# LuoweiZhou/VLP

Hardware: AMD Instinct MI355X
Metric: samples/sec/node (COCO 100-region, seq64, bs64xN) fp16 (higher is better)
Workload: dtype f16; 1 GPU; COCO Captions fine-tune shape: BERT-base 12L, 100 regions x 2048-d, seq_len 64 (L=167), bs 64/GPU, fwd+bwd+FP16 FusedAdam, dropout 0.1, dynamic loss scale; global_batch=64, parallelism=dp1, batch_pool=8, skipped_steps=0, rccl_ranks=1, optimizer=replicated, first_leg_packed=False

## Files before the change

### include/vlp_hip.h

```cpp
#ifndef VLP_HIP_H
#define VLP_HIP_H

#include <stdint.h>

#ifdef __cplusplus
extern "C" {
#endif

#define VLP_ABI_VERSION 5

typedef enum {
    VLP_OK = 0,
    VLP_ERR_BAD_ARG = -1,
    VLP_ERR_HIP = -2,
    VLP_ERR_WORKSPACE = -3
} vlp_status;

enum { VLP_ACT_NONE = 0, VLP_ACT_GELU = 1, VLP_ACT_RELU = 2, VLP_ACT_TANH = 3,
       VLP_ACT_GELU_SAVE_GRAD = 4  };
enum { VLP_MUL_NONE = 0, VLP_MUL_GELU_GRAD = 1, VLP_MUL_RELU_MASK = 2, VLP_MUL_PLAIN = 3  };

int vlp_version(void);
const char* vlp_last_error_string(void);
int vlp_lab_build(void);
// ... 384 lines not shown

int vlp_bce_loss_fwd(const void* logits, int64_t ld, const void* labels_f32, int64_t ldl, int32_t B, int32_t N,
                     float* loss, void* stream);
int vlp_bce_loss_bwd(const void* logits, int64_t ld, const void* labels_f32, int64_t ldl, int32_t B, int32_t N,
                     const float* grad_scale, void* dlogits, int64_t ldd, void* stream);
int vlp_bce_sparse_loss_fwd(const void* logits, int64_t ld, const int32_t* ans_idx, const float* ans_score, int32_t S, int32_t B, int32_t N,
                            float* loss, void* stream);
int vlp_bce_sparse_loss_bwd(const void* logits, int64_t ld, const int32_t* ans_idx, const float* ans_score, int32_t S, int32_t B, int32_t N,
                            const float* grad_scale, void* dlogits, int64_t ldd, void* stream);
int vlp_vqa_answer_rows(const void* logits, int64_t ld, int32_t rows, int32_t N, int32_t first_col, const int32_t* ans_idx,
                        const float* ans_score, int32_t S, int64_t* out_ids, float* out_vals, float* out_scores, void* stream);

int vlp_sumsq(const void* g_f16, int64_t n, float* out2, float* partial, void* stream);
int vlp_sumsq_acc(const void* g_f16, int64_t n, float* out2, float* partial, void* stream);

typedef struct {
    float* p32; float* m; float* v;
    const void* g16;
    void* p16;
    int64_t n;
    float b1, b2, eps, decay;
    int32_t eps_inside_sqrt;
    const float* hyper;
} vlp_fused_adam_args;
int vlp_fused_adam(const vlp_fused_adam_args* a, void* stream);
int vlp_adam_hyper(const float* sumsq2, const float* any_overflow, const float* scale_state, float max_grad_norm,
                   float step_size, float* hyper3, void* stream);
int vlp_loss_scale_update(float* scale_state, const float* overflow, void* stream);

int64_t vlp_bert_adam_norms_floats(int64_t n, int32_t ntensors);
typedef struct {
    float* p32; float* m; float* v;
    const void* g; int32_t g_is_f32;
    void* p16;
    const int64_t* seg_off; int32_t ntensors; int64_t n;
    float* norms; int64_t norms_floats;
    float lr, b1, b2, eps, decay, max_grad_norm;
    float grad_scale;
// ... 9 lines not shown
```

### vlp_amd/_lib.py

```python
import ctypes as C
import os

import torch

_HERE = os.path.dirname(os.path.abspath(__file__))
LIB_PATH = os.environ.get("VLP_HIP_LIB") or os.path.join(_HERE, "libvlp_hip.so")

ACT_NONE, ACT_GELU, ACT_RELU, ACT_TANH, ACT_GELU_SAVE_GRAD = 0, 1, 2, 3, 4
MUL_NONE, MUL_GELU_GRAD, MUL_RELU_MASK, MUL_PLAIN = 0, 1, 2, 3
ROWS_X, ROWS_MUL, ROWS_RES, ROWS_Y = 1, 2, 4, 8

vp, i64, i32, f32, u64, u32 = C.c_void_p, C.c_int64, C.c_int32, C.c_float, C.c_uint64, C.c_uint32


class GemmNtArgs(C.Structure):
    _fields_ = [("X", vp), ("ldx", i64), ("W", vp), ("ldw", i64), ("Y", vp), ("ldy", i64), ("bias", vp),
                ("residual", vp), ("ldr", i64), ("preact", vp), ("ldp", i64), ("mul_src", vp), ("ldm", i64),
                ("M", i32), ("N", i32), ("K", i32), ("act", i32), ("mul_mode", i32), ("alpha", f32),
                ("dropout_p", f32), ("seed", u64), ("rng_stream", u32), ("variant", i32), ("row_map", vp)]


class GemmTnArgs(C.Structure):
    _fields_ = [("A", vp), ("lda", i64), ("B", vp), ("ldb", i64), ("C", vp), ("ldc", i64),
                ("M", i32), ("N", i32), ("K", i32), ("beta", i32), ("workspace", vp), ("workspace_bytes", i64),
# ... 125 lines not shown


class MlmLossBwdArgs(C.Structure):
    _fields_ = [("logits", vp), ("ld_logits", i64), ("labels", vp), ("lse", vp), ("coef", vp), ("grad_scale", vp),
                ("dlogits", vp), ("ld_dlogits", i64), ("rows", i32), ("V", i32)]


class MlmLossLsFwdArgs(C.Structure):
    _fields_ = MlmLossFwdArgs._fields_ + [("smooth", f32), ("confidence", f32), ("q_sum", f32), ("q_log_q", f32), ("ignore_index", i32)]


class MlmLossLsBwdArgs(C.Structure):
    _fields_ = MlmLossBwdArgs._fields_ + [("smooth", f32), ("confidence", f32), ("q_sum", f32), ("ignore_index", i32)]


class FusedAdamArgs(C.Structure):
    _fields_ = [("p32", vp), ("m", vp), ("v", vp), ("g16", vp), ("p16", vp), ("n", i64),
                ("b1", f32), ("b2", f32), ("eps", f32), ("decay", f32), ("eps_inside_sqrt", i32), ("hyper", vp)]


class BertAdamArgs(C.Structure):
    _fields_ = [("p32", vp), ("m", vp), ("v", vp), ("g", vp), ("g_is_f32", i32), ("p16", vp),
                ("seg_off", vp), ("ntensors", i32), ("n", i64), ("norms", vp), ("norms_floats", i64),
                ("lr", f32), ("b1", f32), ("b2", f32), ("eps", f32), ("decay", f32), ("max_grad_norm", f32), ("grad_scale", f32),
                ("active", vp)]


SYMBOLS = {
    "vlp_version": (C.c_int, []),
    "vlp_last_error_string": (C.c_char_p, []),
    "vlp_lab_build": (C.c_int, []),
    "vlp_debug_device_lookup_stats": (None, [vp, vp]),
    "vlp_gemm_nt": (C.c_int, [C.POINTER(GemmNtArgs), vp]),
# ... 769 lines not shown
    _req_cuda(g16, out2, partial)
    fn = load().vlp_sumsq_acc if accumulate else load().vlp_sumsq
    _check(fn(ptr(g16), n, ptr(out2), ptr(partial), stream_ptr()))


def adam_hyper(sumsq2, any_overflow, scale_state, max_grad_norm, step_size, hyper3):
    _req_cuda(sumsq2, hyper3, scale_state)
    _check(load().vlp_adam_hyper(ptr(sumsq2), ptr(any_overflow), ptr(scale_state), max_grad_norm, step_size, ptr(hyper3), stream_ptr()))


def loss_scale_update(scale_state, overflow):
    _req_cuda(scale_state, overflow)
    _check(load().vlp_loss_scale_update(ptr(scale_state), ptr(overflow), stream_ptr()))


def fused_adam(p32, m, v, g16, p16, n, hyper, b1=0.9, b2=0.999, eps=1e-8, decay=0.0, eps_inside_sqrt=False):
    _req_cuda(p32, m, v, g16, p16, hyper)
    a = FusedAdamArgs(ptr(p32), ptr(m), ptr(v), ptr(g16), ptr(p16), n, b1, b2, eps, decay, int(eps_inside_sqrt), ptr(hyper))
    _check(load().vlp_fused_adam(C.byref(a), stream_ptr()))


def bert_adam_norms_floats(n, ntensors):
    return int(load().vlp_bert_adam_norms_floats(n, ntensors))


def bert_adam(p32, m, v, g, g_is_f32, p16, seg_off, ntensors, n, norms, lr, b1=0.9, b2=0.999, eps=1e-6, decay=0.01,
              max_grad_norm=1.0, grad_scale=1.0, active=None):
    _req_cuda(p32, m, v, g, seg_off, norms)
    a = BertAdamArgs(ptr(p32), ptr(m), ptr(v), ptr(g), int(g_is_f32), ptr(p16), ptr(seg_off), ntensors, n, ptr(norms), norms.numel(),
                     lr, b1, b2, eps, decay, max_grad_norm, grad_scale, ptr(active))
    _check(load().vlp_bert_adam(C.byref(a), stream_ptr()))
```

### vlp_amd/csrc/adam.hip

```cpp
#include "common.h"
#include <stdlib.h>

#define SQ_BLOCKS 1024

__global__ __launch_bounds__(256) void sumsq_kernel(const f16* __restrict__ g, int64_t n, float* __restrict__ partial) {
    __shared__ float sh[4], shb[4];
    float s = 0.f, bad = 0.f;
    const int64_t n8 = n >> 3;
    for (int64_t i = (int64_t)blockIdx.x * blockDim.x + threadIdx.x; i < n8; i += (int64_t)gridDim.x * blockDim.x) {
        f16x8 v = ld8(g + i * 8);
#pragma unroll
        for (int e = 0; e < 8; ++e) {
            const float f = (float)v[e];
            s += f * f;
            if (!(fabsf(f) <= 65504.f)) bad = 1.f;
        }
    }
    if (blockIdx.x == 0)
        for (int64_t i = n8 * 8 + threadIdx.x; i < n; i += blockDim.x) {
            const float f = (float)g[i];
            s += f * f;
            if (!(fabsf(f) <= 65504.f)) bad = 1.f;
        }
    s = wave_sum(s);
// ... 77 lines not shown
        }
    }
    if (skip) st[6] += 1.f;
    st[1] += 1.f;
}
extern "C" int vlp_loss_scale_update(float* scale_state, const float* overflow, void* stream) {
    VLP_CHECK_ARG(scale_state && overflow, "vlp_loss_scale_update: bad args");
    VLP_ENTER(scale_state, "vlp_loss_scale_update");
    hipLaunchKernelGGL(loss_scale_update_kernel, dim3(1), dim3(64), 0, (hipStream_t)stream, scale_state, overflow);
    VLP_CHECK_LAUNCH("vlp_loss_scale_update");
    return VLP_OK;
}

DEVFN f32x4 adam_ld4(const float* p) { return __builtin_nontemporal_load(reinterpret_cast<const f32x4*>(p)); }
DEVFN void adam_st4(float* p, f32x4 v) { __builtin_nontemporal_store(v, reinterpret_cast<f32x4*>(p)); }
__global__ __launch_bounds__(256) void fused_adam_kernel(vlp_fused_adam_args a) {
    const float combined = a.hyper[0], step_size = a.hyper[1], skip = a.hyper[2];
    if (skip != 0.f) return;
    const float inv = 1.f / combined;
    const f16* g = (const f16*)a.g16;
    f16* p16 = (f16*)a.p16;
    const int lane = threadIdx.x & 63;
    const int64_t wave = ((int64_t)blockIdx.x * blockDim.x + threadIdx.x) >> 6, nwaves = ((int64_t)gridDim.x * blockDim.x) >> 6;
    for (int64_t base = wave * 512; base < a.n; base += nwaves * 512) {
        f16x4 gv[2];
        f32x4 p0[2], m0[2], v0[2];
        bool ok[2];
#pragma unroll
        for (int h = 0; h < 2; ++h) {
            const int64_t i = base + 256 * h + 4 * lane;
            ok[h] = i < a.n;
            if (ok[h]) {
                gv[h] = __builtin_nontemporal_load(reinterpret_cast<const f16x4*>(g + i));
                p0[h] = adam_ld4(a.p32 + i);
                m0[h] = adam_ld4(a.m + i);
                v0[h] = adam_ld4(a.v + i);
            }
        }
#pragma unroll
        for (int h = 0; h < 2; ++h) {
            if (!ok[h]) continue;
            const int64_t i = base + 256 * h + 4 * lane;
            float pp[4], mm[4], vv[4];
#pragma unroll
            for (int e = 0; e < 4; ++e) { pp[e] = p0[h][e]; mm[e] = m0[h][e]; vv[e] = v0[h][e]; }
            f16x4 o;
#pragma unroll
            for (int e = 0; e < 4; ++e) {
                const float sg = (float)gv[h][e] * inv;
                mm[e] = a.b1 * mm[e] + (1.f - a.b1) * sg;
                vv[e] = a.b2 * vv[e] + (1.f - a.b2) * sg * sg;
                const float denom = a.eps_inside_sqrt ? sqrtf(vv[e] + a.eps) : sqrtf(vv[e]) + a.eps;
                pp[e] = pp[e] - step_size * (mm[e] / denom + a.decay * pp[e]);
                asm volatile("" : "+v"(pp[e]));
                o[e] = (f16)pp[e];
            }
            adam_st4(a.p32 + i, (f32x4){pp[0], pp[1], pp[2], pp[3]});
            adam_st4(a.m + i, (f32x4){mm[0], mm[1], mm[2], mm[3]});
            adam_st4(a.v + i, (f32x4){vv[0], vv[1], vv[2], vv[3]});
            st4(p16 + i, o);
        }
    }
}
extern "C" int vlp_fused_adam(const vlp_fused_adam_args* a, void* stream) {
    VLP_CHECK_ARG(a && a->p32 && a->m && a->v && a->g16 && a->p16 && a->hyper, "vlp_fused_adam: null operand");
    VLP_ENTER(a->p32, "vlp_fused_adam");
    VLP_CHECK_ARG(a->n > 0 && a->n % 8 == 0, "vlp_fused_adam: n must be a positive multiple of 8 (pad the flat buffer)");
    VLP_CHECK_ARG(((uintptr_t)a->p32 | (uintptr_t)a->m | (uintptr_t)a->v | (uintptr_t)a->g16 | (uintptr_t)a->p16) % 16 == 0, "vlp_fused_adam: alignment");
    static const int ncu = [] { int dev = 0, n = 256; (void)hipGetDevice(&dev); if (hipDeviceGetAttribute(&n, hipDeviceAttributeMultiprocessorCount, dev) != hipSuccess) n = 256; return n; }();
    int blocks = (int)((a->n / 8 + 255) / 256);
    if (blocks > 2 * ncu) blocks = 2 * ncu;
    hipLaunchKernelGGL(fused_adam_kernel, dim3(blocks), dim3(256), 0, (hipStream_t)stream, *a);
    VLP_CHECK_LAUNCH("vlp_fused_adam");
    return VLP_OK;
}

#define BA_CHUNK 4096

DEVFN float ba_load(const void* g, int g_is_f32, int64_t i) { return g_is_f32 ? ((const float*)g)[i] : (float)((const f16*)g)[i]; }

DEVFN int ba_find(const int64_t* seg_off, int nt, int64_t i) {
    int lo = 0, hi = nt - 1;
    while (lo < hi) {
        const int mid = (lo + hi + 1) >> 1;
// ... 95 lines not shown
```

### vlp_amd/distributed.py

```python
import os
import time

import torch
import torch.distributed as dist
from torch import nn


class _Stamp(object):

    def __init__(self, cuda):
        self.ev = torch.cuda.Event(enable_timing=True) if cuda else None
        self.t = None

    def record(self, stream=None):
        if self.ev is not None:
            self.ev.record(stream if stream is not None else torch.cuda.current_stream())
        else:
            self.t = time.perf_counter()
        return self

    def ms_until(self, other):
        if self.ev is not None:
            return self.ev.elapsed_time(other.ev)
        return (other.t - self.t) * 1e3
# ... 265 lines not shown


class DistributedDataParallel(nn.Module):

    def __init__(self, module, device_ids=None, output_device=None, find_unused_parameters=False, process_group=None,
                 bucket_cap_mb=50.0, **unused_kwargs):
        super(DistributedDataParallel, self).__init__()
        if not dist.is_initialized():
            raise RuntimeError("init_process_group() must be called before wrapping the model (run_img2txt_dist.py:233)")
        self.module = module
        eng = module.engine
        eng.pack()
        self.engine = eng
        for key in ("decay", "nodecay"):
            dist.broadcast(eng.flat[key], src=0, group=process_group)
        self.reducer = GradReducer(eng.gflat["decay"], eng.buckets, eng.gflat["nodecay"], process_group, bucket_cap_mb)
        eng.grad_ready_hook = self.reducer.bucket_ready
        eng.post_backward_hook = self.reducer.finish
        eng.shard_plan = None
        if self.reducer.mode == "sharded":
            eng.shard_plan = ShardPlan(self.reducer.buckets, eng.gflat["nodecay"].numel(), eng.buckets, self.reducer.world, self.reducer.rank,
                                       process_group)

    def forward(self, *inputs, **kwargs):
        return self.module(*inputs, **kwargs)
```

### vlp_amd/engine.py

```python
import math
import os
import weakref

import numpy as np
import torch

from . import _lib as K
from . import tuning
from .input_prep import MaskSpec, RawRegions, SparseAnswers

ALIGN = 64
NO_DECAY = ("bias", "LayerNorm.bias", "LayerNorm.weight")
PE_DIM = 1607
PE_PAD = 1664


def _ru(x, m):
    return (x + m - 1) // m * m


def is_no_decay(name):
    return any(nd in name for nd in NO_DECAY)


# ... 12 lines not shown
        self.has_mlm = False
        self.pos_ids = None
        self.pk = None
        self.pretext = None
        self.task_labels = None
        self.mlm_smooth = None


class Engine(object):
    GEMM_NT_VARIANT = None
    NT_CANDIDATES = (1, 2, 4, 5, 9, 10, 11, 12, 13, 27, 29, 73, 77, 264)
    NT_CANDIDATES_SKINNY = (1, 2, 9, 10, 11, 17)
    GEMM_TN_VARIANT = 2
    WGRAD_SIDE_STREAM = os.environ.get("VLP_WGRAD_SIDE_STREAM", "1") == "1"
    BLOCK_MASKED_REGION_KEYS = os.environ.get("VLP_BLOCK_MASKED_REGIONS", "0") == "1"
    VARLEN = {"1": True, "0": False}.get(os.environ.get("VLP_VARLEN", ""), "auto")
    TN_SPLITS = None
    TN_VARIANT_CANDIDATES = (2, 26)
    PROF_EVERY = 8
    _nt_choice = {}
    _tn_choice = {}
    _skinny_choice = {}

    def __init__(self, model):
        self._model = weakref.ref(model)
        self.packed = False
        self.gen = 0
        self.step_seed = 0
        self._warned_group_unfused = False
        self.base_seed = 0x5EED
        self.grads_dirty = False
        self.grad_ready_hook = None
        self.post_backward_hook = None
        self.names = self.offsets = self.sizes = self.buckets = None
        self.flat = self.gflat = None
        self._params = None
        self._unused = None
        self._anchor = None
        self.device = None
        self._ws = {}
        self._shadow = None
        self._shadow_ev = None
        self._ln_tab = None
        self._zero1 = None
        self._pretext_on = False
        self._pooler_dirty = False
        self.prof = None
        self._opt_stream = None
        self._param_events = None
        self._params_done = None
        self.shard_plan = None
        self._param_works = None
        self.param_gather_stamps = None
        self._side = None
        self._side_done = None
        self._side_busy = False
        self._prof_ctr = 0
# ... 94 lines not shown
        self._params = params
        self.device = dev
        self.packed = True
        self.grads_dirty = False
        self._anchor = torch.zeros(1, device=dev, requires_grad=True)
        self._unused = set(["bert.pooler.dense.weight", "bert.pooler.dense.bias"])
        if model.tasks == "vqa2":
            self._unused |= {"cls.predictions.bias", "cls.predictions.transform.dense.weight", "cls.predictions.transform.dense.bias",
                             "cls.predictions.transform.LayerNorm.weight", "cls.predictions.transform.LayerNorm.bias"}

    def invalidate(self):
        self.packed = False
        self._ws = {}
        self._shadow = None
        self._shadow_ev = None
        self._ln_tab = None

    def P(self, name):
        return self._params[name].data

    def G(self, name):
        return self._params[name].grad

    def unused_parameter_names(self):
        if self._pretext_on:
            return set(self._unused) - {"bert.pooler.dense.weight", "bert.pooler.dense.bias"}
        return set(self._unused)

    def optimizer_stream(self):
        if self._opt_stream is None:
            self._opt_stream = torch.cuda.Stream(device=self.device)
# ... 127 lines not shown
        self._shadow = sh
        return sh

    def _ln_table(self):
        if self._ln_tab is None:
            NL = self._model().config.num_hidden_layers
            rows = []
            for i in range(NL):
                L = "bert.encoder.layer.%d." % i
                for n in ("attention.output.LayerNorm", "output.LayerNorm"):
                    rows.append([self.G(L + n + ".weight").data_ptr(), self.G(L + n + ".bias").data_ptr()])
            rows.append([self.G("bert.embeddings.LayerNorm.weight").data_ptr(), self.G("bert.embeddings.LayerNorm.bias").data_ptr()])
            self._ln_tab = torch.tensor(rows, dtype=torch.int64, device=self.device)
        return self._ln_tab

    def _refresh_shadows(self):
        sh = self._shadows()
        if "batch" not in sh:
            model = self._model()
            cfg = model.config
            H, I, V = cfg.hidden_size, cfg.intermediate_size, cfg.vocab_size
            items = []
            for i, s in enumerate(sh["layers"]):
                L = "bert.encoder.layer.%d." % i
                items.append((self.P(L + "attention.self.query.weight"), H, s["qkvT"], 3 * H, 3 * H, H, 3 * H))
                items.append((self.P(L + "attention.output.dense.weight"), H, s["oT"], H, H, H, H))
                items.append((self.P(L + "intermediate.dense.weight"), H, s["w1T"], I, I, H, I))
                items.append((self.P(L + "output.dense.weight"), I, s["w2T"], H, H, I, H))
            items.append((self.P("vis_embed.2.weight"), 2048, sh["v2T"], H, H, 2048, H))
            if model.tasks == "vqa2":
                NA = model.num_answers
                items.append((self.P("ans_classifier.2.weight"), 2 * H, sh["a2T"], _ru(NA, 64), NA, 2 * H, _ru(NA, 64)))
                items.append((self.P("ans_classifier.0.weight"), H, sh["a0T"], 2 * H, 2 * H, H, 2 * H))
            else:
                items.append((self.P("cls.predictions.transform.dense.weight"), H, sh["tT"], H, H, H, H))
            sh["batch"] = K.make_transpose_batch(items, self.device)
        K.transpose_batched(sh["batch"])

    def _nt_variant(self, x, w, y, M, N, Kd, kw):
        if self.GEMM_NT_VARIANT is not None:
            return self.GEMM_NT_VARIANT
        key = (M, N, Kd)
        v = Engine._nt_choice.get(key)
        if v is not None:
            return v
        if not tuning.AUTOTUNE:
            v = Engine._nt_choice[key] = tuning.nt_variant(M, N, Kd)
            return v
        best = self.NT_CANDIDATES[0]
        if M * N >= 128 * 128 * 4:
            cands = [c for c in (self.NT_CANDIDATES_SKINNY if M <= 1024 else self.NT_CANDIDATES)
                     if not ((c & 7 == 5 and c < 64 or c == 73) and N < 1024)]
# ... 227 lines not shown
                am = am.to(torch.long).contiguous()
                K.mask_pack(am, ws["maskb"], B, L, ws["Lp"], out_t=want_t)

        self._shadow_ev = None
        pe_ev = mask_ev = None
        if (train or torch.is_grad_enabled()) and self.WGRAD_SIDE_STREAM:
            side = self._side_stream()
            side.wait_stream(torch.cuda.current_stream())
            with torch.cuda.stream(side):
                prep_pe()
                pe_ev = torch.cuda.Event()
                pe_ev.record(side)
                prep_mask(attention_mask)
                mask_ev = torch.cuda.Event()
                mask_ev.record(side)
                if self._params_done is not None:
                    side.wait_event(self._params_done)
                if self._param_works is not None:
                    for w in self._param_works.values():
                        if w is not None:
                            w.wait()
                self._refresh_shadows()
                self._shadow_ev = torch.cuda.Event()
                self._shadow_ev.record(side)
        else:
            prep_mask(attention_mask)
            prep_pe()

        self.wait_params("nodecay")
        self.wait_params(len(self.buckets) - 1)
        self.wait_params(len(self.buckets) - 2)
        self._nt(img, self.P("vis_embed.0.weight"), ws["h1"], Mv, 2048, 2048, bias=self.P("vis_embed.0.bias"), act=K.ACT_RELU)
        self._nt(ws["h1"], self.P("vis_embed.2.weight"), ws["vis_h"], Mv, H, 2048, bias=self.P("vis_embed.2.bias"), act=K.ACT_RELU,
                 dropout_p=p, seed=seed, rng_stream=1001)
        if pe_ev is not None:
            torch.cuda.current_stream().wait_event(pe_ev)
        self._nt(ws["vpe_in"], ws["wpe_pad"], ws["vispe_h"], Mv, H, PE_PAD, bias=self.P("vis_pe_embed.0.bias"), act=K.ACT_RELU,
                 dropout_p=p, seed=seed, rng_stream=1002)
        E = "bert.embeddings."
# ... 613 lines not shown
        B, L, P, ws, seed = st.B, st.L, st.P, st.ws, st.seed
        p, pa = st.p_drop
        M, Mv = B * L, B * Nv
        ro = rm = None
        if st.pk is not None:
            ro, rm, M = st.pk
        beta = 1 if self.grads_dirty else 0
        if beta and self.shard_plan is not None:
            raise RuntimeError("vlp_amd: VLP_DDP_MODE=sharded keeps only this rank's chunk of the reduced gradient, so gradients cannot be "
                               "accumulated over several backward passes (--gradient_accumulation_steps > 1); use allreduce or rs_ag")
        img, input_ids, token_type_ids, masked_pos = st.batch
        self.wait_params()
        if self._shadow_ev is not None:
            torch.cuda.current_stream().wait_event(self._shadow_ev)
            self._shadow_ev = None
        else:
            self._refresh_shadows()
        sh = self._shadows()
        x_last = ws["layers"][NL - 1]["x2"]
        dx = ws["dx"]
        dx.zero_()
        E = "bert.embeddings."
        if beta == 0:
            self.G(E + "position_embeddings.weight").zero_()
            self.G(E + "token_type_embeddings.weight").zero_()

        main = torch.cuda.current_stream()
        use_side = self.WGRAD_SIDE_STREAM
        side = self._side_stream() if use_side else None

        def on_side(fn):
# ... 206 lines not shown
```

### vlp_amd/modeling.py

```python
import copy
import json
import logging
import math
import os
import pickle

import torch
from torch import nn

from . import _lib as K
from .engine import Engine
from .input_prep import MaskSpec, SparseAnswers
from .loss import LabelSmoothingLoss

logger = logging.getLogger(__name__)

CONFIG_NAME = "bert_config.json"
WEIGHTS_NAME = "pytorch_model.bin"
PRETRAINED_MODEL_ARCHIVE_MAP = {
    "bert-base-uncased": None, "bert-large-uncased": None, "bert-base-cased": None, "bert-large-cased": None,
    "bert-base-multilingual-uncased": None, "bert-base-multilingual-cased": None, "bert-base-chinese": None,
}


# ... 255 lines not shown
        if isinstance(module, (nn.Linear, nn.Embedding)):
            module.weight.data.normal_(mean=0.0, std=self.config.initializer_range)
        elif isinstance(module, BertLayerNorm):
            module.bias.data.zero_()
            module.weight.data.fill_(1.0)
        if isinstance(module, nn.Linear) and module.bias is not None:
            module.bias.data.zero_()

    def _apply(self, fn, *a, **k):
        eng = self.__dict__.get("_engine")
        out = super(PreTrainedBertModel, self)._apply(fn, *a, **k)
        if eng is not None:
            eng.invalidate()
        return out

    def __deepcopy__(self, memo):
        cls = self.__class__
        new = cls.__new__(cls)
        memo[id(self)] = new
        for k, v in self.__dict__.items():
            if k == "_engine":
                continue
            new.__dict__[k] = copy.deepcopy(v, memo)
        new.__dict__["_engine"] = Engine(new) if "_engine" in self.__dict__ else None
        for p in new.parameters():
            p.grad = None
            if hasattr(p, "_vlp_engine"):
                del p._vlp_engine
            if new.__dict__["_engine"] is not None:
                p._vlp_owner = new.__dict__["_engine"]
# ... 420 lines not shown
```

### vlp_amd/optimization.py

```python
import math

import torch
from torch.optim import Optimizer
from torch.optim.optimizer import required

from . import _lib as K


def warmup_cosine(x, warmup=0.002):
    if x < warmup:
        return x / warmup
    return 0.5 * (1.0 + math.cos(math.pi * x))


def warmup_constant(x, warmup=0.002):
    if x < warmup:
        return x / warmup
    return 1.0


def warmup_linear(x, warmup=0.002):
    if x < warmup:
        return x / warmup
    return max((x - 1.) / (warmup - 1.), 0)
# ... 127 lines not shown
        eng = self._engine()
        if eng is not None:
            eng.zero_grad()
            return
        for g in self.param_groups:
            for p in g["params"]:
                if p.grad is not None:
                    p.grad.detach_()
                    p.grad.zero_()

    def step(self, closure=None):
        loss = closure() if closure is not None else None
        if self._flat is None:
            self._build()
        eng = self._engine()
        unused = eng.unused_parameter_names() if eng is not None else set()
        name_of = {id(p): n for n, p in eng._params.items()} if eng is not None else {}
        for group, fg in zip(self.param_groups, self._flat):
            act = []
            for i, p in enumerate(fg.params):
                on = p.grad is not None and name_of.get(id(p)) not in unused
                act.append(1 if on else 0)
                if on:
                    fg.g32[fg.offs[i]:fg.offs[i + 1]].copy_(p.grad.detach().reshape(-1))
            if self.grad_scale != 1.0:
                fg.g32.mul_(1.0 / self.grad_scale)
            fg.active.copy_(torch.tensor(act, dtype=torch.int32), non_blocking=True)
            if group["t_total"] != -1:
                lr = group["lr"] * SCHEDULES[group["schedule"]](self._step / group["t_total"], group["warmup"])
            else:
# ... 13 lines not shown
```

### vlp_amd/optimization_fp16.py

```python
import logging
import os

import torch

from . import _lib as K
from .engine import is_no_decay

logger = logging.getLogger(__name__)


class FusedAdam(object):

    def __init__(self, params, lr=1e-3, bias_correction=True, betas=(0.9, 0.999), eps=1e-8, eps_inside_sqrt=False,
                 weight_decay=0., max_grad_norm=0., amsgrad=False):
        if amsgrad:
            raise RuntimeError("FusedAdam does not support the AMSGrad variant.")
        params = list(params)
        if len(params) == 0:
            raise ValueError("optimizer got an empty parameter list")
        if not isinstance(params[0], dict):
            params = [{"params": params}]
        self.defaults = dict(lr=lr, bias_correction=bias_correction, betas=betas, eps=eps, weight_decay=weight_decay, max_grad_norm=max_grad_norm)
        self.param_groups = []
        for g in params:
# ... 148 lines not shown

    def _gather_sharded_state(self):
        plan = getattr(self.engine, "shard_plan", None)
        if plan is None or self._state_gathered_at == self._steps_issued:
            return
        self._state_gathered_at = self._steps_issued
        self.engine.wait_params()
        i_d, i_nd = self._group_key.index("decay"), self._group_key.index("nodecay")
        plan.gather_state([self.fp32_groups_flat[i_d], self._m[i_d], self._v[i_d]], [self.fp32_groups_flat[i_nd], self._m[i_nd], self._v[i_nd]])

    def step(self, closure=None):
        eng = self.engine
        self._steps_issued += 1
        plan = getattr(eng, "shard_plan", None)
        if plan is not None:
            return self._step_sharded(plan)
        if self.pipeline_with_forward:
            return self._step_pipelined()
        eng.wait_params()
        self._grad_norms()
        torch.maximum(self._sumsq[0][1:2], self._sumsq[1][1:2], out=self._ovf)
        for i, key in enumerate(self._group_key):
            g = self.param_groups[i]
            K.adam_hyper(self._sumsq[i], self._ovf, self._scale_state, g["max_grad_norm"], self._step_size(g), self._hyper[i])
            self._adam_range(i, key, 0, eng.sizes[key])
        K.loss_scale_update(self._scale_state, self._ovf)

    def _grad_norms(self):
        eng = self.engine
        for i, key in enumerate(self._group_key):
            K.sumsq(eng.gflat[key], eng.sizes[key], self._sumsq[i], self._partial)

    def _step_size(self, g):
        if g["bias_correction"]:
            b1, b2 = g["betas"]
            t = self.applied_steps + 1
            return g["lr"] * (1 - b2 ** t) ** 0.5 / (1 - b1 ** t)
        return g["lr"]

    def _adam_range(self, i, key, lo, hi):
        g = self.param_groups[i]
        b1, b2 = g["betas"]
        eng = self.engine
        K.fused_adam(self.fp32_groups_flat[i][lo:hi], self._m[i][lo:hi], self._v[i][lo:hi], eng.gflat[key][lo:hi], eng.flat[key][lo:hi], hi - lo,
                     self._hyper[i], b1=b1, b2=b2, eps=g["eps"], decay=g["weight_decay"], eps_inside_sqrt=(self.optimizer.eps_mode == 0))

    def _step_pipelined(self):
        eng = self.engine
        main = torch.cuda.current_stream()
        st = eng.optimizer_stream()
        eng.wait_params()
        st.wait_stream(main)
        events = {}
        with torch.cuda.stream(st):
            self._grad_norms()
            torch.maximum(self._sumsq[0][1:2], self._sumsq[1][1:2], out=self._ovf)
            for i, key in enumerate(self._group_key):
                g = self.param_groups[i]
                K.adam_hyper(self._sumsq[i], self._ovf, self._scale_state, g["max_grad_norm"], self._step_size(g), self._hyper[i])
            i_nd, i_d = self._group_key.index("nodecay"), self._group_key.index("decay")
            self._adam_range(i_nd, "nodecay", 0, eng.sizes["nodecay"])
            ev = torch.cuda.Event()
            ev.record(st)
            events["nodecay"] = ev
            for b in reversed(range(len(eng.buckets))):
                lo, hi = eng.buckets[b]
                self._adam_range(i_d, "decay", lo, hi)
                ev = torch.cuda.Event()
                ev.record(st)
                events[b] = ev
            K.loss_scale_update(self._scale_state, self._ovf)
            done = torch.cuda.Event()
            done.record(st)
        eng.set_param_events(events, done)

    def state_dict(self):
        self._gather_sharded_state()
        self._sync()
        sd = {"dynamic_loss_scale": self.dynamic_loss_scale, "cur_scale": self.cur_scale, "cur_iter": self.cur_iter}
        if self.dynamic_loss_scale:
            sd.update(last_overflow_iter=self.last_overflow_iter, scale_factor=self.scale_factor, scale_window=self.scale_window)
        inner = self.optimizer.state_dict()
        inner["exp_avg"] = [t.clone() for t in self._m]
        inner["exp_avg_sq"] = [t.clone() for t in self._v]
        inner["step"] = self.applied_steps
        inner["group_keys"] = list(self._group_key)
        sd["optimizer_state_dict"] = inner
        sd["fp32_groups_flat"] = [t.clone() for t in self.fp32_groups_flat]
        sd["vlp_rng"] = {"base_seed": self.engine.base_seed, "step_seed": self.engine.step_seed}
# ... 47 lines not shown
        self._scale_state.copy_(st)
        step = 0
        for i, (g, saved) in enumerate(zip(self.param_groups, inner["param_groups"])):
            g.update({k: v for k, v in saved.items() if k != "params"})
            pid = saved["params"][0]
            stt = inner["state"].get(pid) or inner["state"].get(str(pid)) or {}
            if stt:
                self._from_dense(stt["exp_avg"].to(self._m[i].device).float().reshape(-1), self._m[i], i)
                self._from_dense(stt["exp_avg_sq"].to(self._v[i].device).float().reshape(-1), self._v[i], i)
                step = max(step, int(stt.get("step", 0)))
            self._from_dense(sd["fp32_groups_flat"][i].detach().to(self._m[i].device).float().reshape(-1), self.fp32_groups_flat[i], i)
        stl = self._scale_state.tolist()
        self._applied0, self._iter0, self._skipped0 = step, stl[1], stl[6]
        for i, key in enumerate(self._group_key):
            self.engine.flat[key].copy_(self.fp32_groups_flat[i])
        logger.info("FP16_Optimizer_State: resumed from an apex-layout file; the dropout stream position is not part of that layout "
                    "(masks restart from base_seed=%d, step_seed=%d)", self.engine.base_seed, self.engine.step_seed)

    def load_state_dict(self, sd):
        inner = sd.get("optimizer_state_dict", {})
        if "state" in inner and "param_groups" in inner and "exp_avg" not in inner and "group_keys" not in inner:
            return self.load_apex_state_dict(sd)
        self._sync()
        self.dynamic_loss_scale = sd["dynamic_loss_scale"]
        st = self._scale_state.cpu()
        st[0], st[1] = sd["cur_scale"], sd["cur_iter"]
        if sd["dynamic_loss_scale"]:
            st[2], st[3], st[4], st[5] = sd["last_overflow_iter"], sd["scale_factor"], sd["scale_window"], 1.0
        self._scale_state.copy_(st)
        inner = sd["optimizer_state_dict"]
        self.optimizer.load_state_dict(inner)
        for cur, saved in zip(self._m, inner["exp_avg"]):
            cur.copy_(saved)
        for cur, saved in zip(self._v, inner["exp_avg_sq"]):
            cur.copy_(saved)
        st = self._scale_state.tolist()
        self._applied0, self._iter0, self._skipped0 = int(inner.get("step", 0)), st[1], st[6]
        for cur, saved in zip(self.fp32_groups_flat, sd["fp32_groups_flat"]):
            cur.data.copy_(saved.data)
        for i, key in enumerate(self._group_key):
            self.engine.flat[key].copy_(self.fp32_groups_flat[i])
        if "vlp_rng" in sd:
            self.engine.base_seed, self.engine.step_seed = int(sd["vlp_rng"]["base_seed"]), int(sd["vlp_rng"]["step_seed"])
```

Before: 7019 samples/s.

## Fuse transposed fp16 weight shadow writes into the FusedAdam kernel

The Adam update kernel now takes a segment table describing weight matrices that have transposed fp16 shadow copies. For those matrices it processes tiles, stages the updated fp16 values in LDS, and writes the transposed shadow directly. This lets the forward pass skip the separate batched transpose refresh whenever every shadow was covered by the optimizer step. The cost is a more complex tiled kernel with extra shared-memory traffic, plus staleness tracking that has to be invalidated on every parameter load or sharded path.

```diff
diff --git a/include/vlp_hip.h b/include/vlp_hip.h
--- a/include/vlp_hip.h
+++ b/include/vlp_hip.h
@@ -422,6 +422,13 @@
 int vlp_sumsq(const void* g_f16, int64_t n, float* out2, float* partial, void* stream);
 int vlp_sumsq_acc(const void* g_f16, int64_t n, float* out2, float* partial, void* stream);
 
+typedef struct vlp_adam_seg {
+    int64_t off;
+    void* shadow;
+    int64_t ld;
+    int32_t N, K;
+    int32_t tile0, flat0;
+} vlp_adam_seg;
 typedef struct {
     float* p32; float* m; float* v;
     const void* g16;
@@ -430,6 +437,9 @@
     float b1, b2, eps, decay;
     int32_t eps_inside_sqrt;
     const float* hyper;
+    const struct vlp_adam_seg* segs;
+    const struct vlp_adam_seg* segs_host;
+    int32_t nsegs;
 } vlp_fused_adam_args;
 int vlp_fused_adam(const vlp_fused_adam_args* a, void* stream);
 int vlp_adam_hyper(const float* sumsq2, const float* any_overflow, const float* scale_state, float max_grad_norm,
diff --git a/vlp_amd/_lib.py b/vlp_amd/_lib.py
--- a/vlp_amd/_lib.py
+++ b/vlp_amd/_lib.py
@@ -163,9 +163,14 @@
     _fields_ = MlmLossBwdArgs._fields_ + [("smooth", f32), ("confidence", f32), ("q_sum", f32), ("ignore_index", i32)]
 
 
+class AdamSeg(C.Structure):
+    _fields_ = [("off", i64), ("shadow", vp), ("ld", i64), ("N", i32), ("K", i32), ("tile0", i32), ("flat0", i32)]
+
+
 class FusedAdamArgs(C.Structure):
     _fields_ = [("p32", vp), ("m", vp), ("v", vp), ("g16", vp), ("p16", vp), ("n", i64),
-                ("b1", f32), ("b2", f32), ("eps", f32), ("decay", f32), ("eps_inside_sqrt", i32), ("hyper", vp)]
+                ("b1", f32), ("b2", f32), ("eps", f32), ("decay", f32), ("eps_inside_sqrt", i32), ("hyper", vp),
+                ("segs", vp), ("segs_host", vp), ("nsegs", i32)]
 
 
 class BertAdamArgs(C.Structure):
@@ -965,9 +970,29 @@
     _check(load().vlp_loss_scale_update(ptr(scale_state), ptr(overflow), stream_ptr()))
 
 
-def fused_adam(p32, m, v, g16, p16, n, hyper, b1=0.9, b2=0.999, eps=1e-8, decay=0.0, eps_inside_sqrt=False):
+ADAM_TILE_N, ADAM_TILE_K, ADAM_ITEM = 64, 256, 16384
+
+
+def make_adam_segments(items, device):
+    import numpy as np
+    arr = (AdamSeg * max(len(items), 1))()
+    end = tiles = flat = 0
+    for i, (off, N, K, shadow, ld) in enumerate(items):
+        _req_cuda(shadow)
+        arr[i] = AdamSeg(off, shadow.data_ptr(), ld, N, K, tiles, flat)
+        flat += max(0, -(-(off - end) // ADAM_ITEM))
+        tiles += -(-N // ADAM_TILE_N) * -(-K // ADAM_TILE_K)
+        end = off + N * K
+    dev = torch.from_numpy(np.frombuffer(bytes(arr), dtype=np.uint8).copy()).to(device)
+    return arr, dev, len(items)
+
+
+def fused_adam(p32, m, v, g16, p16, n, hyper, b1=0.9, b2=0.999, eps=1e-8, decay=0.0, eps_inside_sqrt=False, segments=None):
     _req_cuda(p32, m, v, g16, p16, hyper)
     a = FusedAdamArgs(ptr(p32), ptr(m), ptr(v), ptr(g16), ptr(p16), n, b1, b2, eps, decay, int(eps_inside_sqrt), ptr(hyper))
+    if segments is not None and segments[2] > 0:
+        host, dev, count = segments
+        a.segs, a.segs_host, a.nsegs = ptr(dev), C.addressof(host), count
     _check(load().vlp_fused_adam(C.byref(a), stream_ptr()))
 
 
diff --git a/vlp_amd/csrc/adam.hip b/vlp_amd/csrc/adam.hip
--- a/vlp_amd/csrc/adam.hip
+++ b/vlp_amd/csrc/adam.hip
@@ -115,53 +115,186 @@
 
 DEVFN f32x4 adam_ld4(const float* p) { return __builtin_nontemporal_load(reinterpret_cast<const f32x4*>(p)); }
 DEVFN void adam_st4(float* p, f32x4 v) { __builtin_nontemporal_store(v, reinterpret_cast<f32x4*>(p)); }
+struct adam_quad { f16x4 g; f32x4 p, m, v; };
+DEVFN void adam_load4(const vlp_fused_adam_args& a, int64_t i, adam_quad& q) {
+    q.g = __builtin_nontemporal_load(reinterpret_cast<const f16x4*>((const f16*)a.g16 + i));
+    q.p = adam_ld4(a.p32 + i);
+    q.m = adam_ld4(a.m + i);
+    q.v = adam_ld4(a.v + i);
+}
+DEVFN f16x4 adam_update4(const vlp_fused_adam_args& a, float inv, float step_size, int64_t i, const adam_quad& q) {
+    float pp[4], mm[4], vv[4];
+#pragma unroll
+    for (int e = 0; e < 4; ++e) { pp[e] = q.p[e]; mm[e] = q.m[e]; vv[e] = q.v[e]; }
+    f16x4 o;
+#pragma unroll
+    for (int e = 0; e < 4; ++e) {
+        const float sg = (float)q.g[e] * inv;
+        mm[e] = a.b1 * mm[e] + (1.f - a.b1) * sg;
+        vv[e] = a.b2 * vv[e] + (1.f - a.b2) * sg * sg;
+        const float denom = a.eps_inside_sqrt ? sqrtf(vv[e] + a.eps) : sqrtf(vv[e]) + a.eps;
+        pp[e] = pp[e] - step_size * (mm[e] / denom + a.decay * pp[e]);
+        asm volatile("" : "+v"(pp[e]));
+        o[e] = (f16)pp[e];
+    }
+    adam_st4(a.p32 + i, (f32x4){pp[0], pp[1], pp[2], pp[3]});
+    adam_st4(a.m + i, (f32x4){mm[0], mm[1], mm[2], mm[3]});
+    adam_st4(a.v + i, (f32x4){vv[0], vv[1], vv[2], vv[3]});
+    st4((f16*)a.p16 + i, o);
+    return o;
+}
 __global__ __launch_bounds__(256) void fused_adam_kernel(vlp_fused_adam_args a) {
     const float combined = a.hyper[0], step_size = a.hyper[1], skip = a.hyper[2];
     if (skip != 0.f) return;
     const float inv = 1.f / combined;
-    const f16* g = (const f16*)a.g16;
-    f16* p16 = (f16*)a.p16;
     const int lane = threadIdx.x & 63;
     const int64_t wave = ((int64_t)blockIdx.x * blockDim.x + threadIdx.x) >> 6, nwaves = ((int64_t)gridDim.x * blockDim.x) >> 6;
     for (int64_t base = wave * 512; base < a.n; base += nwaves * 512) {
-        f16x4 gv[2];
-        f32x4 p0[2], m0[2], v0[2];
+        adam_quad q[2];
         bool ok[2];
 #pragma unroll
         for (int h = 0; h < 2; ++h) {
             const int64_t i = base + 256 * h + 4 * lane;
             ok[h] = i < a.n;
-            if (ok[h]) {
-                gv[h] = __builtin_nontemporal_load(reinterpret_cast<const f16x4*>(g + i));
-                p0[h] = adam_ld4(a.p32 + i);
-                m0[h] = adam_ld4(a.m + i);
-                v0[h] = adam_ld4(a.v + i);
+            if (ok[h]) adam_load4(a, i, q[h]);
+        }
+#pragma unroll
+        for (int h = 0; h < 2; ++h)
+            if (ok[h]) adam_update4(a, inv, step_size, base + 256 * h + 4 * lane, q[h]);
+    }
+}
+
+#define ADAM_TILE_N 64
+#define ADAM_TILE_K 256
+#define ADAM_ITEM 16384
+DEVFN void adam_store_shadow(const uint32_t* T, const vlp_adam_seg& s, int n0, int k0) {
+    f16* sh = (f16*)s.shadow;
+    const bool vec = (s.ld & 7) == 0;
+    const int q8 = threadIdx.x & 7, n = n0 + 8 * q8;
+    if (n >= s.N) return;
+#pragma unroll
+    for (int it = 0; it < 8; ++it) {
+        const int cc = (threadIdx.x >> 3) + 32 * it, k = k0 + cc;
+        if (k >= s.K) break;
+        const f16x8 v = __builtin_bit_cast(f16x8, *reinterpret_cast<const u32x4*>(T + cc * 32 + ((q8 ^ ((cc >> 2) & 7)) << 2)));
+        f16* dst = sh + (int64_t)k * s.ld + n;
+        if (vec && n + 8 <= s.N) __builtin_nontemporal_store(v, reinterpret_cast<f16x8*>(dst));
+        else
+#pragma unroll
+            for (int e = 0; e < 8; ++e) if (n + e < s.N) dst[e] = v[e];
+    }
+}
+__global__ __launch_bounds__(256) void fused_adam_shadow_kernel(vlp_fused_adam_args a, int ntiles, int nitems, int tail_flat0) {
+    __shared__ __attribute__((aligned(16))) uint32_t T[2][ADAM_TILE_K * 32];
+    const float combined = a.hyper[0], step_size = a.hyper[1], skip = a.hyper[2];
+    if (skip != 0.f) return;
+    const float inv = 1.f / combined;
+    const vlp_adam_seg* __restrict__ segs = a.segs;
+    const int nsegs = a.nsegs;
+    const int lane = threadIdx.x & 63, w = threadIdx.x >> 6;
+    int si = 0, gi = 0;
+    int buf = 0, pend = -1, pn0 = 0, pk0 = 0;
+    vlp_adam_seg ps = {};
+    for (int item = blockIdx.x; item < nitems; item += gridDim.x) {
+        if (item < ntiles) {
+            while (si + 1 < nsegs && segs[si + 1].tile0 <= item) ++si;
+            const vlp_adam_seg s = segs[si];
+            const int tiles_k = (s.K + ADAM_TILE_K - 1) / ADAM_TILE_K;
+            const int lt = item - s.tile0;
+            const int n0 = (lt / tiles_k) * ADAM_TILE_N, k0 = (lt % tiles_k) * ADAM_TILE_K;
+            const int c = 4 * lane;
+            const bool cok = k0 + c < s.K;
+            adam_quad q[2];
+            bool ok[2];
+            int64_t i[2];
+            auto load_rows = [&](int j) {
+#pragma unroll
+                for (int h = 0; h < 2; ++h) {
+                    const int r = n0 + 2 * (4 * j + w) + h;
+                    ok[h] = cok && r < s.N;
+                    i[h] = s.off + (int64_t)r * s.K + k0 + c;
+                    if (ok[h]) adam_load4(a, i[h], q[h]);
+                }
+            };
+            load_rows(0);
+            if (pend >= 0) {
+                __syncthreads();
+                adam_store_shadow(T[pend], ps, pn0, pk0);
             }
-        }
-#pragma unroll
-        for (int h = 0; h < 2; ++h) {
-            if (!ok[h]) continue;
-            const int64_t i = base + 256 * h + 4 * lane;
-            float pp[4], mm[4], vv[4];
-#pragma unroll
-            for (int e = 0; e < 4; ++e) { pp[e] = p0[h][e]; mm[e] = m0[h][e]; vv[e] = v0[h][e]; }
-            f16x4 o;
-#pragma unroll
-            for (int e = 0; e < 4; ++e) {
-                const float sg = (float)gv[h][e] * inv;
-                mm[e] = a.b1 * mm[e] + (1.f - a.b1) * sg;
-                vv[e] = a.b2 * vv[e] + (1.f - a.b2) * sg * sg;
-                const float denom = a.eps_inside_sqrt ? sqrtf(vv[e] + a.eps) : sqrtf(vv[e]) + a.eps;
-                pp[e] = pp[e] - step_size * (mm[e] / denom + a.decay * pp[e]);
-                asm volatile("" : "+v"(pp[e]));
-                o[e] = (f16)pp[e];
+            uint32_t* Tb = T[buf];
+#pragma unroll 1
+            for (int j = 0; j < 8; ++j) {
+                if (j > 0) load_rows(j);
+                const int pair = 4 * j + w;
+                f16x4 o[2];
+#pragma unroll
+                for (int h = 0; h < 2; ++h) {
+                    o[h] = (f16x4){0, 0, 0, 0};
+                    if (ok[h]) o[h] = adam_update4(a, inv, step_size, i[h], q[h]);
+                }
+                uint32_t* row = Tb + c * 32 + ((((pair >> 2) ^ (lane & 7)) << 2) | (pair & 3));
+#pragma unroll
+                for (int e = 0; e < 4; ++e) row[e * 32] = __builtin_bit_cast(uint32_t, (f16x2){o[0][e], o[1][e]});
             }
-            adam_st4(a.p32 + i, (f32x4){pp[0], pp[1], pp[2], pp[3]});
-            adam_st4(a.m + i, (f32x4){mm[0], mm[1], mm[2], mm[3]});
-            adam_st4(a.v + i, (f32x4){vv[0], vv[1], vv[2], vv[3]});
-            st4(p16 + i, o);
-        }
-    }
+            pend = buf; ps = s; pn0 = n0; pk0 = k0;
+            buf ^= 1;
+        } else {
+            if (pend >= 0) {
+                __syncthreads();
+                adam_store_shadow(T[pend], ps, pn0, pk0);
+                pend = -1;
+            }
+            const int f = item - ntiles;
+            while (gi < nsegs && (gi + 1 < nsegs ? segs[gi + 1].flat0 : tail_flat0) <= f) ++gi;
+            const int64_t gbeg = gi == 0 ? 0 : segs[gi - 1].off + (int64_t)segs[gi - 1].N * segs[gi - 1].K;
+            const int64_t gend = gi < nsegs ? segs[gi].off : a.n;
+            const int64_t chunk = gbeg + (int64_t)(f - (gi < nsegs ? segs[gi].flat0 : tail_flat0)) * ADAM_ITEM;
+#pragma unroll 1
+            for (int j = 0; j < 8; ++j) {
+                const int64_t base = chunk + (4 * j + w) * 512;
+                if (base >= gend) break;
+                adam_quad q[2];
+                bool ok[2];
+#pragma unroll
+                for (int h = 0; h < 2; ++h) {
+                    const int64_t i = base + 256 * h + 4 * lane;
+                    ok[h] = i < gend;
+                    if (ok[h]) adam_load4(a, i, q[h]);
+                }
+#pragma unroll
+                for (int h = 0; h < 2; ++h)
+                    if (ok[h]) adam_update4(a, inv, step_size, base + 256 * h + 4 * lane, q[h]);
+            }
+        }
+    }
+    if (pend >= 0) {
+        __syncthreads();
+        adam_store_shadow(T[pend], ps, pn0, pk0);
+    }
+}
+static int adam_check_segs(const vlp_fused_adam_args* a, int* ntiles, int* nflat, int* tail_flat0) {
+    VLP_CHECK_ARG(a->nsegs > 0 && a->segs && a->segs_host, "vlp_fused_adam: nsegs = %d needs the table in device (segs) and host (segs_host) memory", (int)a->nsegs);
+    int64_t end = 0, tiles = 0, flat = 0;
+    for (int i = 0; i < a->nsegs; ++i) {
+        const vlp_adam_seg& s = a->segs_host[i];
+        VLP_CHECK_ARG(s.N >= 1 && s.K >= 8 && s.K % 8 == 0, "vlp_fused_adam: segment %d: N = %d, K = %d (N >= 1, K a positive multiple of 8)", i, (int)s.N, (int)s.K);
+        VLP_CHECK_ARG(s.off >= 0 && s.off % 8 == 0 && s.shadow && (uintptr_t)s.shadow % 16 == 0 && s.ld >= s.N,
+                      "vlp_fused_adam: segment %d: offset %lld and shadow must be 16-byte aligned, ld >= N", i, (long long)s.off);
+        VLP_CHECK_ARG(s.off >= end, "vlp_fused_adam: segment %d at %lld overlaps its predecessor (ends at %lld); entries ascend by offset", i, (long long)s.off, (long long)end);
+        VLP_CHECK_ARG(s.off + (int64_t)s.N * s.K <= a->n, "vlp_fused_adam: segment %d [%lld, %lld) leaves [0, n = %lld)", i, (long long)s.off,
+                      (long long)(s.off + (int64_t)s.N * s.K), (long long)a->n);
+        VLP_CHECK_ARG(s.tile0 == tiles && s.flat0 == flat, "vlp_fused_adam: segment %d: tile0 / flat0 = %d / %d, expected %lld / %lld", i, (int)s.tile0, (int)s.flat0,
+                      (long long)tiles, (long long)flat);
+        flat += (s.off - end + ADAM_ITEM - 1) / ADAM_ITEM;
+        tiles += (int64_t)((s.N + ADAM_TILE_N - 1) / ADAM_TILE_N) * ((s.K + ADAM_TILE_K - 1) / ADAM_TILE_K);
+        end = s.off + (int64_t)s.N * s.K;
+    }
+    *tail_flat0 = (int)flat;
+    flat += (a->n - end + ADAM_ITEM - 1) / ADAM_ITEM;
+    VLP_CHECK_ARG(tiles + flat < (1ll << 30), "vlp_fused_adam: too many work items");
+    *ntiles = (int)tiles;
+    *nflat = (int)flat;
+    return VLP_OK;
 }
 extern "C" int vlp_fused_adam(const vlp_fused_adam_args* a, void* stream) {
     VLP_CHECK_ARG(a && a->p32 && a->m && a->v && a->g16 && a->p16 && a->hyper, "vlp_fused_adam: null operand");
@@ -169,6 +302,16 @@
     VLP_CHECK_ARG(a->n > 0 && a->n % 8 == 0, "vlp_fused_adam: n must be a positive multiple of 8 (pad the flat buffer)");
     VLP_CHECK_ARG(((uintptr_t)a->p32 | (uintptr_t)a->m | (uintptr_t)a->v | (uintptr_t)a->g16 | (uintptr_t)a->p16) % 16 == 0, "vlp_fused_adam: alignment");
     static const int ncu = [] { int dev = 0, n = 256; (void)hipGetDevice(&dev); if (hipDeviceGetAttribute(&n, hipDeviceAttributeMultiprocessorCount, dev) != hipSuccess) n = 256; return n; }();
+    if (a->nsegs != 0) {
+        int ntiles = 0, nflat = 0, tail_flat0 = 0;
+        const int rc = adam_check_segs(a, &ntiles, &nflat, &tail_flat0);
+        if (rc != VLP_OK) return rc;
+        int blocks = ntiles + nflat;
+        if (blocks > 2 * ncu) blocks = 2 * ncu;
+        hipLaunchKernelGGL(fused_adam_shadow_kernel, dim3(blocks), dim3(256), 0, (hipStream_t)stream, *a, ntiles, ntiles + nflat, tail_flat0);
+        VLP_CHECK_LAUNCH("vlp_fused_adam(shadows)");
+        return VLP_OK;
+    }
     int blocks = (int)((a->n / 8 + 255) / 256);
     if (blocks > 2 * ncu) blocks = 2 * ncu;
     hipLaunchKernelGGL(fused_adam_kernel, dim3(blocks), dim3(256), 0, (hipStream_t)stream, *a);
diff --git a/vlp_amd/distributed.py b/vlp_amd/distributed.py
--- a/vlp_amd/distributed.py
+++ b/vlp_amd/distributed.py
@@ -303,6 +303,7 @@
         self.engine = eng
         for key in ("decay", "nodecay"):
             dist.broadcast(eng.flat[key], src=0, group=process_group)
+        eng._shadows_current = eng._shadows_valid = False
         self.reducer = GradReducer(eng.gflat["decay"], eng.buckets, eng.gflat["nodecay"], process_group, bucket_cap_mb)
         eng.grad_ready_hook = self.reducer.bucket_ready
         eng.post_backward_hook = self.reducer.finish
diff --git a/vlp_amd/engine.py b/vlp_amd/engine.py
--- a/vlp_amd/engine.py
+++ b/vlp_amd/engine.py
@@ -50,6 +50,7 @@
     GEMM_TN_VARIANT = 2
     WGRAD_SIDE_STREAM = os.environ.get("VLP_WGRAD_SIDE_STREAM", "1") == "1"
     BLOCK_MASKED_REGION_KEYS = os.environ.get("VLP_BLOCK_MASKED_REGIONS", "0") == "1"
+    ADAM_SHADOWS = os.environ.get("VLP_ADAM_SHADOWS", "1") != "0"
     VARLEN = {"1": True, "0": False}.get(os.environ.get("VLP_VARLEN", ""), "auto")
     TN_SPLITS = None
     TN_VARIANT_CANDIDATES = (2, 26)
@@ -77,6 +78,9 @@
         self._ws = {}
         self._shadow = None
         self._shadow_ev = None
+        self._shadows_current = self._shadows_valid = False
+        self._adam_tabs = {}
+        self._adam_covered = 0
         self._ln_tab = None
         self._zero1 = None
         self._pretext_on = False
@@ -201,7 +205,12 @@
         self._ws = {}
         self._shadow = None
         self._shadow_ev = None
+        self._shadows_current = self._shadows_valid = False
+        self._adam_tabs = {}
         self._ln_tab = None
+
+    def shadows_stale(self):
+        self._shadows_current = self._shadows_valid = False
 
     def P(self, name):
         return self._params[name].data
@@ -359,28 +368,61 @@
             self._ln_tab = torch.tensor(rows, dtype=torch.int64, device=self.device)
         return self._ln_tab
 
+    def _shadow_items(self):
+        sh = self._shadows()
+        model = self._model()
+        cfg = model.config
+        H, I = cfg.hidden_size, cfg.intermediate_size
+        items = []
+        for i, s in enumerate(sh["layers"]):
+            L = "bert.encoder.layer.%d." % i
+            items.append((L + "attention.self.query.weight", 3 * H, H, s["qkvT"], 3 * H, 3 * H))
+            items.append((L + "attention.output.dense.weight", H, H, s["oT"], H, H))
+            items.append((L + "intermediate.dense.weight", I, H, s["w1T"], I, I))
+            items.append((L + "output.dense.weight", H, I, s["w2T"], H, H))
+        items.append(("vis_embed.2.weight", H, 2048, sh["v2T"], H, H))
+        if model.tasks == "vqa2":
+            NA = model.num_answers
+            items.append(("ans_classifier.2.weight", NA, 2 * H, sh["a2T"], _ru(NA, 64), _ru(NA, 64)))
+            items.append(("ans_classifier.0.weight", 2 * H, H, sh["a0T"], 2 * H, 2 * H))
+        else:
+            items.append(("cls.predictions.transform.dense.weight", H, H, sh["tT"], H, H))
+        return items
+
     def _refresh_shadows(self):
         sh = self._shadows()
         if "batch" not in sh:
-            model = self._model()
-            cfg = model.config
-            H, I, V = cfg.hidden_size, cfg.intermediate_size, cfg.vocab_size
-            items = []
-            for i, s in enumerate(sh["layers"]):
-                L = "bert.encoder.layer.%d." % i
-                items.append((self.P(L + "attention.self.query.weight"), H, s["qkvT"], 3 * H, 3 * H, H, 3 * H))
-                items.append((self.P(L + "attention.output.dense.weight"), H, s["oT"], H, H, H, H))
-                items.append((self.P(L + "intermediate.dense.weight"), H, s["w1T"], I, I, H, I))
-                items.append((self.P(L + "output.dense.weight"), I, s["w2T"], H, H, I, H))
-            items.append((self.P("vis_embed.2.weight"), 2048, sh["v2T"], H, H, 2048, H))
-            if model.tasks == "vqa2":
-                NA = model.num_answers
-                items.append((self.P("ans_classifier.2.weight"), 2 * H, sh["a2T"], _ru(NA, 64), NA, 2 * H, _ru(NA, 64)))
-                items.append((self.P("ans_classifier.0.weight"), H, sh["a0T"], 2 * H, 2 * H, H, 2 * H))
-            else:
-                items.append((self.P("cls.predictions.transform.dense.weight"), H, sh["tT"], H, H, H, H))
-            sh["batch"] = K.make_transpose_batch(items, self.device)
+            sh["batch"] = K.make_transpose_batch([(self.P(name), cols, dst, ldd, rows, cols, rows_pad)
+                                                  for name, rows, cols, dst, ldd, rows_pad in self._shadow_items()], self.device)
         K.transpose_batched(sh["batch"])
+        self._shadows_current = True
+
+    def adam_segments(self, lo, hi):
+        if not self.ADAM_SHADOWS:
+            return None
+        tab = self._adam_tabs.get((lo, hi))
+        if tab is None:
+            offs, inside = self.offsets["decay"], []
+            for name, rows, cols, dst, ldd, _ in self._shadow_items():
+                off = offs[name]
+                if name.endswith("attention.self.query.weight"):
+                    L = name[:-len("query.weight")]
+                    assert offs[L + "key.weight"] == off + cols * cols and offs[L + "value.weight"] == off + 2 * cols * cols, name
+                assert (lo <= off and off + rows * cols <= hi) or off + rows * cols <= lo or hi <= off, (name, off, rows * cols, lo, hi)
+                if lo <= off and off + rows * cols <= hi:
+                    inside.append((off - lo, rows, cols, dst, ldd))
+            tab = self._adam_tabs[(lo, hi)] = K.make_adam_segments(sorted(inside, key=lambda t: t[0]), self.device)
+        self._adam_covered += tab[2]
+        return tab
+
+    def adam_shadows_begin(self):
+        if self._shadow_ev is not None:
+            torch.cuda.current_stream().wait_event(self._shadow_ev)
+            self._shadow_ev = None
+        self._adam_covered = 0
+
+    def adam_shadows_end(self):
+        self._shadows_valid = self._shadows_current and self._shadow is not None and self._adam_covered == len(self._shadow_items())
 
     def _nt_variant(self, x, w, y, M, N, Kd, kw):
         if self.GEMM_NT_VARIANT is not None:
@@ -638,15 +680,16 @@
                 prep_mask(attention_mask)
                 mask_ev = torch.cuda.Event()
                 mask_ev.record(side)
-                if self._params_done is not None:
-                    side.wait_event(self._params_done)
-                if self._param_works is not None:
-                    for w in self._param_works.values():
-                        if w is not None:
-                            w.wait()
-                self._refresh_shadows()
-                self._shadow_ev = torch.cuda.Event()
-                self._shadow_ev.record(side)
+                if not self._shadows_valid:
+                    if self._params_done is not None:
+                        side.wait_event(self._params_done)
+                    if self._param_works is not None:
+                        for w in self._param_works.values():
+                            if w is not None:
+                                w.wait()
+                    self._refresh_shadows()
+                    self._shadow_ev = torch.cuda.Event()
+                    self._shadow_ev.record(side)
         else:
             prep_mask(attention_mask)
             prep_pe()
@@ -1290,7 +1333,7 @@
         if self._shadow_ev is not None:
             torch.cuda.current_stream().wait_event(self._shadow_ev)
             self._shadow_ev = None
-        else:
+        elif not self._shadows_valid:
             self._refresh_shadows()
         sh = self._shadows()
         x_last = ws["layers"][NL - 1]["x2"]
diff --git a/vlp_amd/modeling.py b/vlp_amd/modeling.py
--- a/vlp_amd/modeling.py
+++ b/vlp_amd/modeling.py
@@ -293,6 +293,12 @@
             eng.invalidate()
         return out
 
+    def load_state_dict(self, *a, **k):
+        eng = self.__dict__.get("_engine")
+        if eng is not None:
+            eng.shadows_stale()
+        return super(PreTrainedBertModel, self).load_state_dict(*a, **k)
+
     def __deepcopy__(self, memo):
         cls = self.__class__
         new = cls.__new__(cls)
diff --git a/vlp_amd/optimization.py b/vlp_amd/optimization.py
--- a/vlp_amd/optimization.py
+++ b/vlp_amd/optimization.py
@@ -165,6 +165,8 @@
         if self._flat is None:
             self._build()
         eng = self._engine()
+        if eng is not None:
+            eng.shadows_stale()
         unused = eng.unused_parameter_names() if eng is not None else set()
         name_of = {id(p): n for n, p in eng._params.items()} if eng is not None else {}
         for group, fg in zip(self.param_groups, self._flat):
diff --git a/vlp_amd/optimization_fp16.py b/vlp_amd/optimization_fp16.py
--- a/vlp_amd/optimization_fp16.py
+++ b/vlp_amd/optimization_fp16.py
@@ -186,17 +186,20 @@
         self._steps_issued += 1
         plan = getattr(eng, "shard_plan", None)
         if plan is not None:
+            eng.shadows_stale()
             return self._step_sharded(plan)
         if self.pipeline_with_forward:
             return self._step_pipelined()
         eng.wait_params()
         self._grad_norms()
         torch.maximum(self._sumsq[0][1:2], self._sumsq[1][1:2], out=self._ovf)
+        eng.adam_shadows_begin()
         for i, key in enumerate(self._group_key):
             g = self.param_groups[i]
             K.adam_hyper(self._sumsq[i], self._ovf, self._scale_state, g["max_grad_norm"], self._step_size(g), self._hyper[i])
-            self._adam_range(i, key, 0, eng.sizes[key])
+            self._adam_range(i, key, 0, eng.sizes[key], shadows=True)
         K.loss_scale_update(self._scale_state, self._ovf)
+        eng.adam_shadows_end()
 
     def _grad_norms(self):
         eng = self.engine
@@ -210,12 +213,13 @@
             return g["lr"] * (1 - b2 ** t) ** 0.5 / (1 - b1 ** t)
         return g["lr"]
 
-    def _adam_range(self, i, key, lo, hi):
+    def _adam_range(self, i, key, lo, hi, shadows=False):
         g = self.param_groups[i]
         b1, b2 = g["betas"]
         eng = self.engine
+        seg = eng.adam_segments(lo, hi) if shadows and key == "decay" else None
         K.fused_adam(self.fp32_groups_flat[i][lo:hi], self._m[i][lo:hi], self._v[i][lo:hi], eng.gflat[key][lo:hi], eng.flat[key][lo:hi], hi - lo,
-                     self._hyper[i], b1=b1, b2=b2, eps=g["eps"], decay=g["weight_decay"], eps_inside_sqrt=(self.optimizer.eps_mode == 0))
+                     self._hyper[i], b1=b1, b2=b2, eps=g["eps"], decay=g["weight_decay"], eps_inside_sqrt=(self.optimizer.eps_mode == 0), segments=seg)
 
     def _step_pipelined(self):
         eng = self.engine
@@ -231,13 +235,14 @@
                 g = self.param_groups[i]
                 K.adam_hyper(self._sumsq[i], self._ovf, self._scale_state, g["max_grad_norm"], self._step_size(g), self._hyper[i])
             i_nd, i_d = self._group_key.index("nodecay"), self._group_key.index("decay")
+            eng.adam_shadows_begin()
             self._adam_range(i_nd, "nodecay", 0, eng.sizes["nodecay"])
             ev = torch.cuda.Event()
             ev.record(st)
             events["nodecay"] = ev
             for b in reversed(range(len(eng.buckets))):
                 lo, hi = eng.buckets[b]
-                self._adam_range(i_d, "decay", lo, hi)
+                self._adam_range(i_d, "decay", lo, hi, shadows=True)
                 ev = torch.cuda.Event()
                 ev.record(st)
                 events[b] = ev
@@ -245,6 +250,7 @@
             done = torch.cuda.Event()
             done.record(st)
         eng.set_param_events(events, done)
+        eng.adam_shadows_end()
 
     def state_dict(self):
         self._gather_sharded_state()
@@ -322,6 +328,7 @@
         self._applied0, self._iter0, self._skipped0 = step, stl[1], stl[6]
         for i, key in enumerate(self._group_key):
             self.engine.flat[key].copy_(self.fp32_groups_flat[i])
+        self.engine.shadows_stale()
         logger.info("FP16_Optimizer_State: resumed from an apex-layout file; the dropout stream position is not part of that layout "
                     "(masks restart from base_seed=%d, step_seed=%d)", self.engine.base_seed, self.engine.step_seed)
 
@@ -348,5 +355,6 @@
             cur.data.copy_(saved.data)
         for i, key in enumerate(self._group_key):
             self.engine.flat[key].copy_(self.fp32_groups_flat[i])
+        self.engine.shadows_stale()
         if "vlp_rng" in sd:
             self.engine.base_seed, self.engine.step_seed = int(sd["vlp_rng"]["base_seed"]), int(sd["vlp_rng"]["step_seed"])
```

Measured after the change: 6986 samples/s. Within noise of the previous version (-0.5%).
